# gillesdegottex/percivaltts

Hardware: AMD Instinct MI355X
Metric: acoustic frames/sec per WGAN-GP critic+gen step (higher is better)
Workload: dtype f32

## Files before the change

### include/percival_hip.h

```cpp
#ifndef PERCIVAL_HIP_H
#define PERCIVAL_HIP_H

#include <stddef.h>
#include <stdint.h>

#ifdef __cplusplus
extern "C" {
#endif

#define PTTS_OK            0
#define PTTS_EINVAL       -1
#define PTTS_ELAUNCH      -2
#define PTTS_EWORKSPACE   -3
#define PTTS_EDEVICE      -4

#define PTTS_IN_NONE     0
#define PTTS_IN_LRELU    1
#define PTTS_IN_MASKMUL  2

#define PTTS_PAD_SAME    0
#define PTTS_PAD_CAUSAL  1

#define PTTS_ACT_NONE    0
#define PTTS_ACT_LRELU   1
// ... 126 lines not shown
                                     int Kin, int N, int M, long long lda, long long ldb, int in_mode, float alpha,
                                     void* stream);
int ptts_dense_wgrad_reduce_grouped(const ptts_dense_wgrad_reduce_desc* descs, int n, void* stream);
int ptts_dense_wgrad_bf16x6(const float* A, const float* dY, const float* mask_src, const float* in_scale,
                            const float* in_shift, float* C, float* colsum_b, void* workspace, size_t workspace_bytes,
                            int Kin, int N, int M, long long lda, long long ldb, long long ldc, int in_mode, float alpha,
                            void* stream);
int ptts_dense_bf16x6(const float* A, const void* planes, const float* bias, float* C, int M, int N, int K,
                      long long lda, long long ldc, int in_mode, const float* in_scale, const float* in_shift,
                      const float* mask_src, float alpha, int accumulate, const float* out_mask, void* stream);
int ptts_dense_bf16x6_res(const float* A, const void* planes, const float* bias, float* C, int M, int N, int K,
                          long long lda, long long ldc, int in_mode, const float* in_scale, const float* in_shift,
                          const float* mask_src, float alpha, const float* res, int res_rows, long long ldr,
                          const float* out_mask, void* stream);
int ptts_dense_bf16x6_stats_rows(int M, int N);
int ptts_dense_bf16x6_stats(const float* A, const void* planes, const float* bias, float* C, int M, int N, int K,
                            long long lda, long long ldc, int in_mode, const float* in_scale, const float* in_shift,
                            float alpha, double* stats, int capacity_rows, int* nrows_out, void* stream);
int ptts_dense_bf16x6_bwd_affine(const float* A, const void* planes, float* C, int M, int N, int K, long long lda, long long ldc,
                                 const float* z, const float* scale, const float* shift, float alpha,
                                 double* stats, int capacity_rows, int* nrows_out, void* stream);
int ptts_partial_rows_sum(const double* partials, int nrows, int ncols, double* out, void* stream);
int ptts_dft_mirror(float* Ap, int NB, int B, int Cin, int Kh, void* stream);

int ptts_conv1d_freq_kernel_planes(const float* w, const float* tw, void* planes, int NB, int KW, int Cin, int N, int Kh, void* stream);

int ptts_transpose_batched(const float* src, float* dst, int nb, int rows, int cols, void* stream);
int ptts_conv1d_freq_wgrad_combine(const float* out2, float* dW, int KW, int Cin, int N, int Kh, void* stream);

size_t ptts_conv1d_freq_wgrad_inverse_workspace_bytes(int KW, int Cin, int N);
int ptts_conv1d_freq_wgrad_inverse(const float* Gt, const float* t2, float* dW, void* workspace, size_t workspace_bytes,
                                   int NB, int NBp, int KW, int Cin, int N, int Kh, void* stream);

int ptts_dense_bf16x6_batched(const float* A, long long strideA, const void* planes, long long stride_planes_bytes,
                              const float* bias, float* C, long long strideC, int nbatch, int M, int N, int K,
                              long long lda, long long ldc, int planes_count, void* stream);

int ptts_split3_frames(const float* x, void* p1, void* p2, void* p3, int B, int T, int C, int pad_left, int pad_right,
                       int Cp, void* stream);
int ptts_split3_weight_t(const float* w, void* p1, void* p2, void* p3, int KW, int C, int N, int Cp, void* stream);
int ptts_conv1d_bf16x6(const void* a1, const void* a2, const void* a3, const void* bt1, const void* bt2, const void* bt3,
                       const float* bias, float* y, int B, int T, int KW, int Cp, int N, void* stream);

int ptts_split3_frames_t(const float* x, void* p1, void* p2, void* p3, int B, int T, int C, int pad_left, int Tp, int Crows,
                         long long Pp, void* stream);
int ptts_conv1d_wgrad_bf16x6(const void* xt1, const void* xt2, const void* xt3, const void* yt1, const void* yt2,
                             const void* yt3, float* dw, int B, int T, int KW, int C, int N, int Crows, long long Pp,
                             void* stream);

int ptts_transpose_frames(const float* x, float* out, int B, int T, int C, int pad_left, int Tp, int Crows, long long Pp,
                          void* stream);
int ptts_conv1d_wgrad_t(const float* xt, const float* yt, float* dw, float* db, int B, int T, int KW, int C, int N, int Crows,
                        long long Pp, void* stream);

size_t ptts_colstats_workspace_bytes(long long rows, int C);
int ptts_colstats(const float* x, long long rows, int C,
                  int in_mode, const float* in_scale, const float* in_shift, const float* mask_src, float alpha,
                  double* sums , void* workspace, size_t workspace_bytes, void* stream);

int ptts_bn_finalize(const double* sums, long long count, const float* gamma, const float* beta,
                     float* moving_mean, float* moving_var, float eps, float momentum,
                     int training, int update_moving, int unbiased_moving, int C,
                     float* scale, float* shift, float* mean , float* rstd , void* stream);

int ptts_bn_batch_stats_supported(long long rows, int C);
int ptts_bn_batch_stats(const float* x, long long rows, int C, const float* gamma, const float* beta,
// ... 134 lines not shown
```

### percivaltts_amd/csrc/dense.hip

```cpp
#include "common.h"
#include <cstdlib>

namespace ptts {
namespace dns {

typedef __bf16 bf16x8 __attribute__((ext_vector_type(8)));
typedef __bf16 bf16x4 __attribute__((ext_vector_type(4)));
typedef __bf16 bf16x2 __attribute__((ext_vector_type(2)));
typedef float f32x4 __attribute__((ext_vector_type(4)));
typedef float f32x2 __attribute__((ext_vector_type(2)));
typedef unsigned u32x2 __attribute__((ext_vector_type(2)));
typedef unsigned short u16;

constexpr int THREADS = 512;
constexpr int NBLK = 256;
constexpr int BK = 32;

#define DNS_PRODUCTS(X) X(2, 0) X(1, 1) X(0, 2) X(1, 0) X(0, 1) X(0, 0)
#define DNS_PRODUCTS_NPL(NPL, X) do { if (NPL == 3) { X(2, 0) X(1, 1) X(0, 2) X(1, 0) X(0, 1) } X(0, 0) } while (0)

__device__ __forceinline__ unsigned pk_bf16(float a, float b) {
    return __builtin_bit_cast(unsigned, __builtin_convertvector((f32x2){a, b}, bf16x2));
}
__device__ __forceinline__ void split3_pair(float a, float b, unsigned& p1, unsigned& p2, unsigned& p3) {
    p1 = pk_bf16(a, b);
    const float ra = a - __builtin_bit_cast(float, p1 << 16), rb = b - __builtin_bit_cast(float, p1 & 0xffff0000u);
    p2 = pk_bf16(ra, rb);
    const float sa = ra - __builtin_bit_cast(float, p2 << 16), sb = rb - __builtin_bit_cast(float, p2 & 0xffff0000u);
    p3 = pk_bf16(sa, sb);
}
__device__ __forceinline__ float max_fast(float a, float b) {
    float r;
    asm("v_max_f32 %0, %1, %2" : "=v"(r) : "v"(a), "v"(b));
    return r;
}

__global__ __launch_bounds__(256) void split3_dense_weight_kernel(const float* __restrict__ w, long long ldw, int K, int N,
                                                                  int transposed, u16* __restrict__ planes, int NT, int KS) {
    const long long idx = (long long)blockIdx.x * 256 + threadIdx.x;
    if (idx >= (long long)NT * KS * 64) return;
    const int lane = (int)(idx & 63);
    const long long t = idx >> 6;
    const int ks = (int)(t % KS), nt = (int)(t / KS);
    const int n = nt * 16 + (lane & 15), k0 = ks * 32 + (lane >> 4) * 8;
// ... 151 lines not shown
    const int li = lane & 15, lg = lane >> 4;
#pragma unroll
    for (int j = 0; j < 4; ++j) {
        const int ntl = wave + 4 * j;
        const int nt = cb * 16 + ntl;
        if (nt >= a.NT) continue;
        float v[8];
#pragma unroll
        for (int e = 0; e < 8; ++e) v[e] = tile[(8 * lg + e) * SPL_ROW + 16 * ntl + li];
        unsigned q[3][4];
#pragma unroll
        for (int h = 0; h < 4; ++h) split3_pair(v[2 * h], v[2 * h + 1], q[0][h], q[1][h], q[2][h]);
        const size_t idx = ((size_t)nt * a.KS + ks) * 64 + lane;
#pragma unroll
        for (int p = 0; p < 3; ++p)
            *reinterpret_cast<uint4*>(planes + p * ps + idx * 8) = make_uint4(q[p][0], q[p][1], q[p][2], q[p][3]);
    }
}

#ifndef DNS_DEPTH
#define DNS_DEPTH 2
#endif
struct DenseArgs {
    const float* A; const float* mask_src; const float* in_scale; const float* in_shift;
    const u16* planes; const float* bias; const float* out_mask; float* C;
    int M, N, K, NT, KS;
    long long lda, ldc;
    float alpha, out_alpha;
    int accumulate, has_affine, vec_out;
    const float* res; int res_rows; long long ldr;
    long long bsA, bsP, bsC;
    double* stats;
    const float* om_scale; const float* om_shift;
};

template <int MODE, bool AFFINE, int MT, int NPL>
__global__ __launch_bounds__(THREADS) void dense_bf16x6_kernel(DenseArgs g) {
    if (gridDim.z > 1) {
        g.A += (long long)blockIdx.z * g.bsA;
        g.planes += (long long)blockIdx.z * g.bsP;
        g.C += (long long)blockIdx.z * g.bsC;
    }
    constexpr int TBM = 16 * MT;
    constexpr int NA = (TBM * 8 + THREADS - 1) / THREADS;
    constexpr int ROWS = NA * THREADS / 8;
    constexpr int PL = ROWS * BK;
    constexpr bool MASK = MODE == PTTS_IN_MASKMUL;
    __shared__ __attribute__((aligned(16))) u16 As[2][NPL * PL];
    const int tid = threadIdx.x, lane = tid & 63;
    const int wave = __builtin_amdgcn_readfirstlane(tid >> 6);
    const int li = lane & 15, lg = lane >> 4;
    const int m0 = blockIdx.x * TBM, n0 = blockIdx.y * NBLK;
    const int KS = g.KS;
    const bool wave_live = n0 + 32 * wave < g.N;

    const int kq = tid & 7;
    const float* pa[NA]; const float* pm[NA]; bool oka[NA]; int dst[NA];
#pragma unroll
    for (int j = 0; j < NA; ++j) {
        const int row = (tid + j * THREADS) >> 3;
        oka[j] = row < TBM && m0 + row < g.M;
        const long long base = (long long)(oka[j] ? m0 + row : 0) * g.lda + 4 * kq;
        pa[j] = g.A + base;
        pm[j] = MASK ? g.mask_src + base : nullptr;
        dst[j] = row * BK + ((((kq >> 1) ^ ((row >> 1) & 2))) << 3) + (kq & 1) * 4;
    }
    struct Stage { f32x4 va[NA], vm[MASK ? NA : 1], sc, sh; bool kok; };
    auto load_a = [&](int s, Stage& sg) {
        const int k = s * BK + 4 * kq;
        sg.kok = k < g.K;
        const int ko = sg.kok ? s * BK : -4 * kq;
#pragma unroll
        for (int j = 0; j < NA; ++j) {
            sg.va[j] = *reinterpret_cast<const f32x4*>(pa[j] + ko);
            if (MASK) sg.vm[j] = *reinterpret_cast<const f32x4*>(pm[j] + ko);
        }
        if (AFFINE) {
            sg.sc = *reinterpret_cast<const f32x4*>(g.in_scale + (sg.kok ? k : 0));
            sg.sh = *reinterpret_cast<const f32x4*>(g.in_shift + (sg.kok ? k : 0));
        }
    };
    auto commit = [&](const Stage& sg, u16* as) {
        const f32x4 z4 = {0.f, 0.f, 0.f, 0.f};
#pragma unroll
        for (int j = 0; j < NA; ++j) {
            f32x4 a = sg.va[j];
            if (MODE == PTTS_IN_LRELU) {
                if (AFFINE) a = a * sg.sc + sg.sh;
                if (!(oka[j] && sg.kok)) a = z4;
#pragma unroll
                for (int e = 0; e < 4; ++e) a[e] = max_fast(a[e], g.alpha * a[e]);
            } else if (MASK) {
                if (!(oka[j] && sg.kok)) a = z4;
#pragma unroll
                for (int e = 0; e < 4; ++e) a[e] = a[e] * (sg.vm[j][e] > 0.f ? 1.f : g.alpha);
            } else {
                if (!(oka[j] && sg.kok)) a = z4;
            }
            u16* d = as + dst[j];
            if (NPL == 3) {
                unsigned a1, a2, a3, b1, b2, b3;
                split3_pair(a[0], a[1], a1, a2, a3);
                split3_pair(a[2], a[3], b1, b2, b3);
                *reinterpret_cast<u32x2*>(d) = (u32x2){a1, b1};
                *reinterpret_cast<u32x2*>(d + PL) = (u32x2){a2, b2};
                *reinterpret_cast<u32x2*>(d + 2 * PL) = (u32x2){a3, b3};
            } else {
                *reinterpret_cast<u32x2*>(d) = (u32x2){pk_bf16(a[0], a[1]), pk_bf16(a[2], a[3])};
            }
        }
    };

    const size_t ps = (size_t)g.NT * KS * 512;
    const u16* wp[2];
#pragma unroll
    for (int j = 0; j < 2; ++j) wp[j] = g.planes + (((size_t)((n0 >> 4) + 2 * (wave_live ? wave : 0) + j) * KS) * 64 + lane) * 8;
    auto load_w = [&](int s, bf16x8 (&wf)[2][NPL]) {
#pragma unroll
        for (int j = 0; j < 2; ++j)
#pragma unroll
            for (int p = 0; p < NPL; ++p) wf[j][p] = *reinterpret_cast<const bf16x8*>(wp[j] + p * ps + (size_t)s * 512);
    };

    f32x4 acc[MT][2];
#pragma unroll
    for (int i = 0; i < MT; ++i) { acc[i][0] = f32x4{0.f, 0.f, 0.f, 0.f}; acc[i][1] = f32x4{0.f, 0.f, 0.f, 0.f}; }
    const int boff = li * BK + ((lg ^ ((li >> 1) & 2)) << 3);
    auto mfma_rows = [&](const u16* as, const bf16x8 (&wf)[2][NPL], int i0, int i1) {
#pragma unroll
        for (int i = i0; i < i1; ++i) {
            bf16x8 bf[NPL];
#pragma unroll
            for (int p = 0; p < NPL; ++p) bf[p] = *reinterpret_cast<const bf16x8*>(as + p * PL + boff + i * 16 * BK);
#define DNS_MM(PA, PW)                                                                                    \
            acc[i][0] = __builtin_amdgcn_mfma_f32_16x16x32_bf16(wf[0][PW < NPL ? PW : 0], bf[PA < NPL ? PA : 0], acc[i][0], 0, 0, 0);    \
            acc[i][1] = __builtin_amdgcn_mfma_f32_16x16x32_bf16(wf[1][PW < NPL ? PW : 0], bf[PA < NPL ? PA : 0], acc[i][1], 0, 0, 0);
            DNS_PRODUCTS_NPL(NPL, DNS_MM);
#undef DNS_MM
        }
    };

    constexpr int DEPTH = DNS_DEPTH;
    Stage sg[DEPTH];
    bf16x8 wc[2][NPL], wn[2][NPL];
#pragma unroll
    for (int j = 0; j < DEPTH; ++j) load_a(j, sg[j]);
    load_w(0, wc);
    commit(sg[0], As[0]);
    load_a(DEPTH, sg[0]);
    __syncthreads();
    auto step = [&](int s, int cut, Stage& nx) {
        const u16* as = As[s & 1];
        load_w(s + 1 < KS ? s + 1 : s, wn);
        mfma_rows(as, wc, 0, cut);
        commit(nx, As[(s + 1) & 1]);
        load_a(s + 1 + DEPTH, nx);
        mfma_rows(as, wc, cut, MT);
#pragma unroll
        for (int j = 0; j < 2; ++j)
#pragma unroll
            for (int p = 0; p < NPL; ++p) wc[j][p] = wn[j][p];
        __syncthreads();
    };
    auto run = [&](int cut) {
        int s = 0;
        for (; s + DEPTH <= KS; s += DEPTH) {
#pragma unroll
            for (int j = 0; j < DEPTH; ++j) step(s + j, cut, sg[(j + 1) % DEPTH]);
        }
#pragma unroll
        for (int j = 0; j < DEPTH; ++j)
            if (s + j < KS) step(s + j, cut, sg[(j + 1) % DEPTH]);
    };
    if (wave < 4) run(2); else run(MT - 2);
    if (!wave_live) return;
    const bool interior = m0 + TBM <= g.M;
    if (!g.vec_out) {
#pragma unroll
        for (int j = 0; j < 2; ++j)
#pragma unroll
            for (int i = 0; i < MT; ++i) {
                const int m = m0 + 16 * i + li;
                if (m >= g.M) continue;
#pragma unroll
                for (int e = 0; e < 4; ++e) {
// ... 455 lines not shown
}
extern "C" int ptts_dense_bf16x6_stats_rows(int M, int N) {
    if (M <= 0 || N <= 0) return 0;
    const int mt = pick_mt(M, (N + NBLK - 1) / NBLK);
    return (M + 16 * mt - 1) / (16 * mt);
}

static int dense_launch(const float* A, const void* planes, const float* bias, float* C, int M, int N, int K,
                        long long lda, long long ldc, int in_mode, const float* in_scale, const float* in_shift,
                        const float* mask_src, float alpha, const float* res, int res_rows, long long ldr,
                        const float* out_mask, double* stats, int stats_capacity_rows, int* stats_rows_out, void* stream) {
    const int accumulate = res != nullptr;
    PTTS_REQUIRE(!res || (res_rows > 0 && ldr >= N && M <= 8LL * res_rows), "dense_bf16x6: bad residual (rows %d, ldr %lld)", res_rows, ldr);
    PTTS_REQUIRE(A && planes && C, "dense_bf16x6: null matrix");
    PTTS_REQUIRE(ptts_dense_bf16x6_supported(M, N, K, lda, ldc), "dense_bf16x6: unsupported shape M=%d N=%d K=%d lda=%lld ldc=%lld (K and lda must be multiples of 4)", M, N, K, lda, ldc);
    PTTS_REQUIRE(lda >= K && ldc >= N, "dense_bf16x6: bad leading dims");
    PTTS_REQUIRE(in_mode >= 0 && in_mode <= 2, "dense_bf16x6: bad in_mode %d", in_mode);
    PTTS_REQUIRE((in_scale == nullptr) == (in_shift == nullptr), "dense_bf16x6: scale/shift must come together");
    PTTS_REQUIRE(in_mode != PTTS_IN_MASKMUL || mask_src, "dense_bf16x6: MASKMUL needs mask_src");
    PTTS_REQUIRE(in_mode == PTTS_IN_LRELU || !in_scale, "dense_bf16x6: scale/shift need PTTS_IN_LRELU");
    PTTS_REQUIRE(!(out_mask && bias), "dense_bf16x6: out_mask with bias is not defined");
    PTTS_REQUIRE(alpha >= 0.f && alpha <= 1.f, "dense_bf16x6: LeakyReLU slope %g outside [0, 1]", alpha);
    const bool vec_out = N % 4 == 0 && ldc % 4 == 0 && ((uintptr_t)C & 15) == 0 && (!bias || ((uintptr_t)bias & 15) == 0) &&
                         (!out_mask || ((uintptr_t)out_mask & 15) == 0) && (!res || (((uintptr_t)res & 15) == 0 && ldr % 4 == 0));
    PTTS_REQUIRE(((uintptr_t)A & 15) == 0 && (!mask_src || ((uintptr_t)mask_src & 15) == 0) &&
                 (!in_scale || (((uintptr_t)in_scale | (uintptr_t)in_shift) & 15) == 0), "dense_bf16x6: A, its mask and scale/shift must be 16-byte aligned");
    DenseArgs g;
    g.A = A; g.mask_src = mask_src; g.in_scale = in_scale; g.in_shift = in_shift; g.planes = (const u16*)planes; g.bias = bias;
    g.out_mask = out_mask; g.C = C; g.M = M; g.N = N; g.K = K;
    g.NT = (N + NBLK - 1) / NBLK * (NBLK / 16); g.KS = (K + BK - 1) / BK;
    g.lda = lda; g.ldc = ldc; g.alpha = alpha; g.out_alpha = alpha; g.accumulate = accumulate; g.has_affine = in_scale != nullptr; g.vec_out = vec_out;
    g.res = res; g.res_rows = res ? res_rows : 1; g.ldr = ldr;
    g.bsA = g.bsP = g.bsC = 0;
    const int cb = (N + NBLK - 1) / NBLK;
    const int mt = pick_mt(M, cb);
    const dim3 grid((unsigned)((M + 16 * mt - 1) / (16 * mt)), (unsigned)cb);
    g.stats = stats;
    g.om_scale = g_om_scale; g.om_shift = g_om_shift;
    if (stats) {
        PTTS_REQUIRE(vec_out, "dense_bf16x6_stats: N and ldc must be multiples of 4, C (and bias) 16-byte aligned");
        PTTS_REQUIRE(stats_capacity_rows >= (int)grid.x, "dense_bf16x6_stats: room for %d rows of sums, %d needed", stats_capacity_rows, (int)grid.x);
        *stats_rows_out = (int)grid.x;
    }
    hipStream_t st = (hipStream_t)stream;
    const bool one = ptts::bf16_products();
#define DNS_L(MODE, AFF, MT) do { if (one) hipLaunchKernelGGL((dense_bf16x6_kernel<MODE, AFF, MT, 1>), grid, dim3(THREADS), 0, st, g); \
                                  else hipLaunchKernelGGL((dense_bf16x6_kernel<MODE, AFF, MT, 3>), grid, dim3(THREADS), 0, st, g); } while (0)
#define DNS_M(MT)                                                                \
    do {                                                                         \
        if (in_mode == PTTS_IN_LRELU) { if (in_scale) DNS_L(PTTS_IN_LRELU, true, MT); else DNS_L(PTTS_IN_LRELU, false, MT); } \
        else if (in_mode == PTTS_IN_MASKMUL) DNS_L(PTTS_IN_MASKMUL, false, MT);  \
        else DNS_L(PTTS_IN_NONE, false, MT);                                     \
    } while (0)
    switch (mt) {
        case 4: DNS_M(4); break;
        case 5: DNS_M(5); break;
        case 6: DNS_M(6); break;
        case 7: DNS_M(7); break;
        default: DNS_M(8); break;
    }
#undef DNS_M
#undef DNS_L
    return check_launch("dense_bf16x6");
}

extern "C" int ptts_conv1d_freq_kernel_planes(const float* w, const float* tw, void* planes, int NB, int KW, int Cin, int N, int Kh,
                                              void* stream) {
    PTTS_REQUIRE(w && tw && planes && NB > 0 && Cin > 0 && N > 0, "conv1d_freq_kernel_planes: bad arguments");
    PTTS_REQUIRE(Kh >= Cin && Kh % 8 == 0, "conv1d_freq_kernel_planes: Kh=%d must be a multiple of 8 and >= Cin=%d", Kh, Cin);
    const int NT = (N + NBLK - 1) / NBLK * (NBLK / 16), KS = (2 * Kh + BK - 1) / BK;
    const long long total = (long long)NT * KS * 64;
    const long long fstride = (long long)(ptts_dense_planes_bytes(N, 2 * Kh) / sizeof(u16));
    const dim3 grid((unsigned)((total + 255) / 256), (unsigned)((NB + WDFT_FCH - 1) / WDFT_FCH));
#define WDFT(KWv) hipLaunchKernelGGL(conv1d_wdft_planes_kernel<KWv>, grid, dim3(256), 0, (hipStream_t)stream, w, tw, (u16*)planes, fstride, NB, Cin, N, Kh, NT, KS)
    switch (KW) {
        case 3: WDFT(3); break;
        case 5: WDFT(5); break;
        case 7: WDFT(7); break;
        case 9: WDFT(9); break;
        case 11: WDFT(11); break;
        case 21: WDFT(21); break;
        default: set_error("conv1d_freq_kernel_planes: KW=%d not instantiated (3, 5, 7, 9, 11, 21)", KW); return PTTS_EINVAL;
    }
#undef WDFT
    return check_launch("conv1d_freq_kernel_planes");
}

extern "C" int ptts_dense_bf16x6_batched(const float* A, long long strideA, const void* planes, long long stride_planes_bytes,
                                         const float* bias, float* C, long long strideC, int nbatch, int M, int N, int K,
                                         long long lda, long long ldc, int planes_count, void* stream) {
    PTTS_REQUIRE(A && planes && C && nbatch > 0 && nbatch <= 65535, "dense_bf16x6_batched: bad arguments");
    PTTS_REQUIRE(ptts_dense_bf16x6_supported(M, N, K, lda, ldc), "dense_bf16x6_batched: unsupported shape M=%d N=%d K=%d lda=%lld ldc=%lld", M, N, K, lda, ldc);
    PTTS_REQUIRE(lda >= K && ldc >= N && planes_count >= 1 && planes_count <= 3 && planes_count != 2, "dense_bf16x6_batched: bad leading dims / planes");
    PTTS_REQUIRE(stride_planes_bytes % 16 == 0 && strideA % 4 == 0 && ((uintptr_t)A & 15) == 0, "dense_bf16x6_batched: strides of A / planes must keep 16-byte alignment");
    const bool vec_out = N % 4 == 0 && ldc % 4 == 0 && strideC % 4 == 0 && ((uintptr_t)C & 15) == 0 && (!bias || ((uintptr_t)bias & 15) == 0);
    DenseArgs g;
    g.A = A; g.mask_src = nullptr; g.in_scale = nullptr; g.in_shift = nullptr; g.planes = (const u16*)planes; g.bias = bias;
    g.out_mask = nullptr; g.C = C; g.M = M; g.N = N; g.K = K;
    g.NT = (N + NBLK - 1) / NBLK * (NBLK / 16); g.KS = (K + BK - 1) / BK;
    g.lda = lda; g.ldc = ldc; g.alpha = 0.f; g.out_alpha = 0.f; g.accumulate = 0; g.has_affine = 0; g.vec_out = vec_out;
    g.res = nullptr; g.res_rows = 1; g.ldr = 0;
    g.bsA = strideA; g.bsP = stride_planes_bytes / 2; g.bsC = strideC;
    g.stats = nullptr; g.om_scale = g.om_shift = nullptr;
    const int cb = (N + NBLK - 1) / NBLK;
    int mt = 8; double best_eff = -1.0;
    {
        static int forced = -1;
        if (forced < 0) { const char* e = getenv("PTTS_DENSE_BATCHED_MT"); forced = e ? atoi(e) : 0; }
        for (int m = 8; m >= 4; --m) {
            const int tiles = (M + 16 * m - 1) / (16 * m);
            const double eff = (double)M / (double)(tiles * 16 * m);
            if (eff > best_eff + 1e-9) { best_eff = eff; mt = m; }
        }
        if (forced >= 4 && forced <= 8) mt = forced;
    }
    const dim3 grid((unsigned)((M + 16 * mt - 1) / (16 * mt)), (unsigned)cb, (unsigned)nbatch);
    hipStream_t st = (hipStream_t)stream;
    const bool one = planes_count == 1;
#define DNS_B(MT) do { if (one) hipLaunchKernelGGL((dense_bf16x6_kernel<PTTS_IN_NONE, false, MT, 1>), grid, dim3(THREADS), 0, st, g); \
                       else hipLaunchKernelGGL((dense_bf16x6_kernel<PTTS_IN_NONE, false, MT, 3>), grid, dim3(THREADS), 0, st, g); } while (0)
    switch (mt) {
        case 4: DNS_B(4); break;
        case 5: DNS_B(5); break;
        case 6: DNS_B(6); break;
        case 7: DNS_B(7); break;
        default: DNS_B(8); break;
    }
#undef DNS_B
    return check_launch("dense_bf16x6_batched");
}

extern "C" int ptts_dense_wgrad_bf16x6_supported(int Kin, int N, int M, long long lda, long long ldb) {
    return (Kin > 0 && N > 0 && M > 0 && Kin % 4 == 0 && N % 4 == 0 && lda % 4 == 0 && ldb % 4 == 0 &&
            (long long)((Kin + WT - 1) / WT) * ((N + WT - 1) / WT) <= 65535) ? 1 : 0;
}

namespace {
int wgrad_split(int Kin, int N, int M) {
    const int tiles = ((Kin + WT - 1) / WT) * ((N + WT - 1) / WT), steps = (M + 31) / 32;
    int split = (256 + tiles - 1) / tiles;
    static int env_split = -1;
    if (env_split < 0) { const char* e = getenv("PTTS_DENSE_WGRAD_SPLIT"); env_split = e ? atoi(e) : 0; }
    if (env_split > 0) split = env_split;
    if (split > steps) split = steps;
    return split < 1 ? 1 : split;
}
}

extern "C" size_t ptts_dense_wgrad_workspace_bytes(int Kin, int N, int M) {
    if (Kin <= 0 || N <= 0 || M <= 0) return 0;
    const size_t tiles = (size_t)((Kin + WT - 1) / WT) * ((N + WT - 1) / WT);
    return tiles * wgrad_split(Kin, N, M) * WPART * sizeof(float);
}

extern "C" int ptts_dense_wgrad_bf16x6_partials(const float* A, const float* dY, const float* mask_src, const float* in_scale,
                                                const float* in_shift, void* workspace, size_t workspace_bytes, int* split_out,
                                                int Kin, int N, int M, long long lda, long long ldb, int in_mode, float alpha,
                                                void* stream) {
    PTTS_REQUIRE(A && dY && workspace && split_out, "dense_wgrad_bf16x6: null pointer");
    PTTS_REQUIRE(ptts_dense_wgrad_bf16x6_supported(Kin, N, M, lda, ldb), "dense_wgrad_bf16x6: unsupported shape Kin=%d N=%d M=%d lda=%lld ldb=%lld", Kin, N, M, lda, ldb);
    PTTS_REQUIRE(lda >= Kin && ldb >= N, "dense_wgrad_bf16x6: bad leading dims");
// ... 73 lines not shown
```

### percivaltts_amd/ops.py

```python
import contextlib
import ctypes
import os

import torch

from . import _hip
from ._hip import call, ptr, stream, f32c, _workspace
from .ops_offline import *

IN_NONE, IN_LRELU, IN_MASKMUL = 0, 1, 2
PAD_SAME, PAD_CAUSAL = 0, 1
ACT_NONE, ACT_LRELU, ACT_SIGMOID, ACT_TANH = 0, 1, 2, 3
ACT_CODES = {None: ACT_NONE, 'linear': ACT_NONE, 'lrelu': ACT_LRELU, 'sigmoid': ACT_SIGMOID, 'tanh': ACT_TANH}


class Lazy(object):
    __slots__ = ('z', 'scale', 'shift', 'lrelu', 'alpha')

    def __init__(self, z, scale=None, shift=None, lrelu=False, alpha=0.3):
        self.z, self.scale, self.shift, self.lrelu, self.alpha = z, scale, shift, lrelu, alpha

    @property
    def shape(self):
        return self.z.shape

    def tensor(self):
        if self.scale is None and not self.lrelu:
            return self.z
        return affine_act(self.z, self.scale, self.shift, 'lrelu' if self.lrelu else None, self.alpha)


def as_lazy(v):
    return v if isinstance(v, Lazy) else Lazy(v)


def as_tensor(v):
    return v.tensor() if isinstance(v, Lazy) else v


def _fusable(lz):
    if lz.lrelu:
        return IN_LRELU, lz.scale, lz.shift
    if lz.scale is None:
# ... 1257 lines not shown
        Crows = (C + 63) // 64 * 64
        key = None if src is None else (src._version, tuple(src.shape), KW, _hip.stream_id())
        if src is not None and cls.src is src and cls.key == key:
            return cls.planes
        xt = torch.empty((Crows, Pp), dtype=torch.float32, device=ap.device)
        call('ptts_transpose_frames', ptr(ap), ptr(xt), B, Tp, C, 0, Tp, Crows, Pp, stream(), tag=(B, Tp, C))
        out = (xt, Crows, Pp)
        if src is not None:
            cls.src, cls.key, cls.planes = src, key, out
        return out

    @classmethod
    def clear(cls):
        cls.src = cls.key = cls.planes = None


def clear_caches():
    _C1Split.clear()
    _C1FFT.clear()
    _C1WgradT.clear()
    _C2M.clear()
    _C2C.clear()
    _DenseSplit.clear()
    _C1Cache.key = _C1Cache.ap = _C1Cache.y = None


class _C1FFT(object):
    default = os.environ.get('PTTS_CONV1D_FFT', '1') == '1'
    enabled = default
    KWS = (3, 5, 7, 9, 11, 21)
    wgrad_enabled = os.environ.get('PTTS_CONV1D_FFT_WGRAD', '1') == '1'
    bf16_one_product = os.environ.get('PTTS_CONV1D_FFT_BF16', '1') == '1'
    seg_target = int(os.environ.get('PTTS_CONV1D_FFT_SEG', '100'))
    consts = {}
    x_src = None; x_key = None; x_hat = None
    xw_src = None; xw_key = None; xw_planes = None
    w_hat = {}
    bufs = {}

    @staticmethod
    def eligible(a, w):
        B, T, Cin = a.shape
        KW, _, N = w.shape
        if not (a.is_cuda and B * T >= 4096 and KW >= 3 and KW % 2 == 1 and T % 4 == 0 and N % 4 == 0 and Cin >= 64):
            return False
        return B * (T // _C1FFT.segment(T, KW)) <= 65535

    @classmethod
    def segment(cls, T, KW):
        tgt = cls.seg_target
        if tgt <= 0:
            return T
        best = T
        for S in range(4, T + 1, 4):
            if T % S == 0 and S >= 2 * KW and abs(S - tgt) < abs(best - tgt):
                best = S
        return best

    @classmethod
    def _buf(cls, name, key, nfloats, dev):
        sid = _hip.stream_id()
        k = (name, key, sid)
        t = cls.bufs.get(k)
        if t is None:
            for k2 in [k2 for k2 in cls.bufs if k2[0] == name and k2[2] == sid]:
                del cls.bufs[k2]
            t = cls.bufs[k] = torch.zeros(nfloats, dtype=torch.float32, device=dev)
        return t

    @classmethod
    def _scratch(cls, name, nbytes, dev):
        k = ('scratch', name, _hip.stream_id())
        t = cls.bufs.get(k)
        if t is None or t.numel() < nbytes:
            t = cls.bufs[k] = torch.empty(int(nbytes), dtype=torch.uint8, device=dev)
        return t

    @classmethod
    def const(cls, T, KW, Cin, dev):
# ... 12 lines not shown
        th = 2.0 * math.pi * torch.remainder(f * i, P) / P
        D = torch.stack([torch.cos(th), -torch.sin(th)], dim=1).reshape(2 * NB, P)
        cf = torch.full((NB,), 2.0, dtype=torch.float64); cf[0] = 1.0; cf[P // 2] = 1.0
        R = 2 * NB
        Rp = (R + 3) // 4 * 4
        E = torch.zeros(S, Rp, dtype=torch.float64)
        E[:, 0:R:2] = (torch.cos(th[:, :S]) * cf.view(NB, 1) / P).t()
        E[:, 1:R:2] = (-torch.sin(th[:, :S]) * cf.view(NB, 1) / P).t()
        k = torch.arange(KW, dtype=torch.float64).view(1, KW)
        tk = 2.0 * math.pi * torch.remainder(f * k, P) / P
        Tw = torch.stack([torch.cos(tk), torch.sin(tk)], dim=1).reshape(R, KW)
        NBp = (NB + 3) // 4 * 4
        T2 = torch.zeros(2 * KW, NBp, dtype=torch.float64)
        T2[:KW, :NB] = (torch.cos(tk) * cf.view(NB, 1) / P).t()
        T2[KW:, :NB] = (torch.sin(tk) * cf.view(NB, 1) / P).t()
        TP = (2 * KW + 15) // 16 * 16
        T2f = torch.zeros(NB, TP, dtype=torch.float64)
        T2f[:, :2 * KW] = T2[:, :NB].t()
        to = lambda m: m.to(torch.float32).to(dev).contiguous()
        c = {'S': S, 'NS': NS, 'P': P, 'NB': NB, 'R': R, 'Rp': Rp, 'NBp': NBp, 'TP': TP, 'pl': pl, 'Kh': (Cin + 7) // 8 * 8,
             'D': to(D), 'E': to(E), 'Tw': to(Tw), 'T2': to(T2), 'T2f': to(T2f)}
        cls.consts[key] = c
        return c

    @classmethod
    def x_transform(cls, a, KW):
        B, T, Cin = a.shape
        key = (a._version, tuple(a.shape), KW, _hip.stream_id())
        if cls.x_src is a and cls.x_key == key:
            return cls.x_hat
        c = cls.const(T, KW, Cin, a.device)
        NB, Kh, NS, S, P = c['NB'], c['Kh'], c['NS'], c['S'], c['P']
        Z = B * NS
        Ap = cls._buf('Ap', (B, T, Cin, KW, S), NB * 2 * Z * 2 * Kh, a.device)
        lib = _hip.lib()
        npb = lib.ptts_dense_planes_bytes(Cin, P)
        xpl = cls._scratch('xpl', Z * npb, a.device)
        call('ptts_split3_frame_windows', ptr(a), B, T, Cin, NS, S, -c['pl'], P, P, ptr(xpl), npb, stream(), tag=('x', Z))
        call('ptts_dense_bf16x6_batched', ptr(c['D']), 0, ptr(xpl), npb, None, ptr(Ap), 2 * Kh, Z, c['R'], Cin, P, P, Z * 2 * Kh, 3, stream(),
             tag=('dft', Z, c['R'], Cin, P))
        call('ptts_dft_mirror', ptr(Ap), NB, Z, Cin, Kh, stream())
        cls.x_src, cls.x_key, cls.x_hat = a, key, Ap
        return Ap

    @classmethod
    def kernel(cls, w, T):
        KW, Cin, N = w.shape
        flat = getattr(w, '_ptts_flat', None)
        epoch = None if flat is None else flat.epoch
        sid = _hip.stream_id()
        c = cls.const(T, KW, Cin, w.device)
        NB, Kh = c['NB'], c['Kh']
        geo = (c['S'], NB, Kh)
        ent = cls.w_hat.get((id(w), sid))
        if ent is not None and ent[0] is w and ent[1] == w._version and ent[2] == epoch and flat is not None and ent[5] == geo:
            if cls.frozen_log is not None and id(flat) in cls.frozen:
                cls.frozen_log.append((w, ent[4], T))
            return ent[4]
        lib = _hip.lib()
        npb = lib.ptts_dense_planes_bytes(N, 2 * Kh)
        if ent is not None and ent[0] is w and ent[5] == geo:
            planes = ent[4]
        else:
            planes = torch.empty(NB * npb, dtype=torch.uint8, device=w.device)
        cls._build_kernel_planes(w, c, planes)
        if len(cls.w_hat) >= 8 and (id(w), sid) not in cls.w_hat:
            cls.w_hat = {k: e for k, e in cls.w_hat.items() if id(getattr(e[0], '_ptts_flat', None)) in cls.frozen}
        cls.w_hat[(id(w), sid)] = (w, w._version, epoch, None, planes, geo, T)
        return planes

    @classmethod
    def _build_kernel_planes(cls, w, c, planes):
        KW, Cin, N = w.shape
        NB, Kh = c['NB'], c['Kh']
        if KW in cls.KWS:
            call('ptts_conv1d_freq_kernel_planes', ptr(w), ptr(c['Tw']), ptr(planes), NB, KW, Cin, N, Kh, stream(), tag=(NB, KW, Cin, N))
        else:
            npb = _hip.lib().ptts_dense_planes_bytes(N, 2 * Kh)
            What = torch.zeros(c['R'] * Kh * N, dtype=torch.float32, device=w.device)
            gemm_raw(c['Tw'], w.view(KW, Cin * N), What, c['R'], Cin * N, KW, lda=KW, ldb=Cin * N, ldc=Kh * N)
            call('ptts_split3_dense_weight_strided', ptr(What), 2 * Kh * N, ptr(planes), npb, NB, N, 2 * Kh, N, 0, stream(), tag=('w', NB))

    frozen = set()
    frozen_log = None

    @classmethod
    def refresh_planes(cls, items):
        for w, planes, T in items:
            KW, Cin, N = w.shape
            cls._build_kernel_planes(w, cls.const(T, KW, Cin, w.device), planes)
        return len(items)

    @classmethod
    def forward(cls, a, w, b, y):
        B, T, Cin = a.shape
        KW, _, N = w.shape
        c = cls.const(T, KW, Cin, a.device)
        NB, Kh, NS, S = c['NB'], c['Kh'], c['NS'], c['S']
        Z = B * NS
        lib = _hip.lib()
        Ap = cls.x_transform(a, KW)
        wpl = cls.kernel(w, T)
        npw = lib.ptts_dense_planes_bytes(N, 2 * Kh)
        Yh = cls._scratch('Yh', NB * 2 * Z * N * 4, a.device)
        call('ptts_dense_bf16x6_batched', ptr(Ap), 2 * Z * 2 * Kh, ptr(wpl), npw, None, ptr(Yh), 2 * Z * N, NB, 2 * Z, N, 2 * Kh,
             2 * Kh, N, 1 if _Flags.bf16_products else 3, stream(), tag=('freq', NB, 2 * Z, N, 2 * Kh))
        npy = lib.ptts_dense_planes_bytes(N, c['R'])
        ypl = cls._scratch('ypl', Z * npy, a.device)
        call('ptts_split3_dense_weight_strided', ptr(Yh), N, ptr(ypl), npy, Z, Z * N, c['R'], N, 0, stream(), tag=('y', Z))
        call('ptts_dense_bf16x6_batched', ptr(c['E']), 0, ptr(ypl), npy, ptr(b), ptr(y), S * N, Z, S, N, c['Rp'], c['Rp'], N, 3, stream(),
             tag=('idft', Z, S, N, c['Rp']))

    @classmethod
    def has_x(cls, a, KW):
        return a is not None and cls.x_src is a and cls.x_key == (a._version, tuple(a.shape), KW, _hip.stream_id())

    @classmethod
    def wgrad(cls, a, dy, KW):
        B, T, Cin = a.shape
        N = dy.shape[-1]
        c = cls.const(T, KW, Cin, a.device)
        NB, Kh, NS, S, P = c['NB'], c['Kh'], c['NS'], c['S'], c['P']
        Z = B * NS
        lib = _hip.lib()
        dev = a.device
        Ap = cls.x_hat
        npx = lib.ptts_dense_planes_bytes(2 * Kh, 2 * Z)
        if cls.xw_src is not a or cls.xw_key != cls.x_key or cls.xw_planes is None:
            xw = cls._scratch('xw', NB * npx, dev)
            call('ptts_split3_dense_weight_strided', ptr(Ap), 2 * Z * 2 * Kh, ptr(xw), npx, NB, 2 * Kh, 2 * Z, 2 * Kh, 0, stream(), tag=('xw', NB))
            cls.xw_src, cls.xw_key, cls.xw_planes = a, cls.x_key, xw
        npd = lib.ptts_dense_planes_bytes(N, P)
        dpl = cls._scratch('dpl', Z * npd, dev)
        call('ptts_split3_frame_windows', ptr(dy), B, T, N, NS, S, 0, P, S, ptr(dpl), npd, stream(), tag=('dy', Z))
        DYh = cls._scratch('DYh', NB * 2 * Z * N * 4, dev)
        call('ptts_dense_bf16x6_batched', ptr(c['D']), 0, ptr(dpl), npd, None, ptr(DYh), N, Z, c['R'], N, P, P, Z * N, 3, stream(),
             tag=('dft_dy', Z, c['R'], N, P))
        DYt = cls._scratch('DYt', NB * N * 2 * Z * 4, dev)
        call('ptts_transpose_batched', ptr(DYh), ptr(DYt), NB, 2 * Z, N, stream())
        Gt = cls._scratch('Gt', NB * N * 2 * Kh * 4, dev)
        call('ptts_dense_bf16x6_batched', ptr(DYt), N * 2 * Z, ptr(cls.xw_planes), npx, None, ptr(Gt), N * 2 * Kh, NB, N, 2 * Kh, 2 * Z,
             2 * Z, 2 * Kh, 1 if _Flags.bf16_products else 3, stream(), tag=('corr', NB, N, 2 * Kh, 2 * Z))
        dw = torch.empty((KW, Cin, N), dtype=torch.float32, device=dev)
        if KW in cls.KWS:
            ws = _workspace(lib.ptts_conv1d_freq_wgrad_inverse_workspace_bytes(KW, Cin, N), dev)
            call('ptts_conv1d_freq_wgrad_inverse', ptr(Gt), ptr(c['T2f']), ptr(dw), ptr(ws), ws.numel(), NB, c['TP'], KW, Cin, N, Kh, stream(),
                 tag=(NB, KW, Cin, N))
        else:
            out2 = torch.empty(2 * KW * N * 2 * Kh, dtype=torch.float32, device=dev)
            gemm_raw(c['T2'], Gt[:NB * N * 2 * Kh * 4].view(torch.float32), out2, 2 * KW, N * 2 * Kh, NB, lda=c['NBp'], ldb=N * 2 * Kh, ldc=N * 2 * Kh)
            call('ptts_conv1d_freq_wgrad_combine', ptr(out2), ptr(dw), KW, Cin, N, Kh, stream())
        return dw

    @classmethod
    def clear(cls):
        cls.x_src = cls.x_key = cls.x_hat = None
        cls.xw_src = cls.xw_key = cls.xw_planes = None
        cls.w_hat = {k: (e if id(getattr(e[0], '_ptts_flat', None)) in cls.frozen else (e[0], None, None, e[3], e[4], e[5]) + tuple(e[6:]))
                     for k, e in cls.w_hat.items()}


def conv1d_fft(on):
    _C1FFT.enabled = _C1FFT.default if on is None else bool(on)
    _C1FFT.clear()


def conv1d_split(on):
    _C1Split.enabled = _C1Split.default if on is None else bool(on)
    _C1Split.clear()


class Conv1dFn(torch.autograd.Function):
    @staticmethod
    def forward(ctx, a, w, b, pre=None):
        f32c(a, 'conv1d.a'); f32c(w, 'conv1d.w')
        B, T, Cin = a.shape
        KW, Ci2, N = w.shape
        assert Ci2 == Cin
        pl = (KW - 1) // 2
        if pre is not None:
            saved, padded, y = pre
        else:
            y = torch.empty((B, T, N), dtype=torch.float32, device=a.device)
            if _C1FFT.enabled and _C1Split.enabled and (not _Flags.bf16_products or _C1FFT.bf16_one_product) and _C1FFT.eligible(a, w):
                _C1FFT.forward(a, w, b, y)
                saved, padded = a, False
            elif _C1Split.enabled and not _Flags.deterministic and _C1Split.eligible(a, w):
                xp, Cp = _C1Split.frames(a, pl, KW - 1 - pl)
                wp = _C1Split.kernel(w)
# ... 683 lines not shown
```

Before: 4.563 million.

## Store DFT spectra compactly and synthesize mirrored half inside dense GEMM loads

Adds left- and right-mirrored operand forms to the batched bf16x6 dense kernel. The kernel reconstructs the sign-flipped mirrored half of the frequency-domain input on the fly, either while loading A or by offsetting and flipping the weight planes. The FFT conv1d path then stores only half the spectrum when the batch-segment count is a multiple of 32, which skips the dft_mirror pass and halves the Ap buffer and xw plane split. In exchange it adds per-load branching, sign XORs and extra template instantiations in the hot GEMM loops.

After: 4.138 million. -9.3%, worse.

```diff
diff --git a/include/percival_hip.h b/include/percival_hip.h
--- a/include/percival_hip.h
+++ b/include/percival_hip.h
@@ -182,6 +182,8 @@
 int ptts_conv1d_freq_wgrad_inverse(const float* Gt, const float* t2, float* dW, void* workspace, size_t workspace_bytes,
                                    int NB, int NBp, int KW, int Cin, int N, int Kh, void* stream);
 
+#define PTTS_DENSE_LEFT_MIRRORED  0x100
+#define PTTS_DENSE_RIGHT_MIRRORED 0x200
 int ptts_dense_bf16x6_batched(const float* A, long long strideA, const void* planes, long long stride_planes_bytes,
                               const float* bias, float* C, long long strideC, int nbatch, int M, int N, int K,
                               long long lda, long long ldc, int planes_count, void* stream);
diff --git a/percivaltts_amd/csrc/dense.hip b/percivaltts_amd/csrc/dense.hip
--- a/percivaltts_amd/csrc/dense.hip
+++ b/percivaltts_amd/csrc/dense.hip
@@ -10,6 +10,7 @@
 typedef float f32x4 __attribute__((ext_vector_type(4)));
 typedef float f32x2 __attribute__((ext_vector_type(2)));
 typedef unsigned u32x2 __attribute__((ext_vector_type(2)));
+typedef unsigned u32x4 __attribute__((ext_vector_type(4)));
 typedef unsigned short u16;
 
 constexpr int THREADS = 512;
@@ -227,9 +228,10 @@
     long long bsA, bsP, bsC;
     double* stats;
     const float* om_scale; const float* om_shift;
+    int mirZ, mirKh;
 };
 
-template <int MODE, bool AFFINE, int MT, int NPL>
+template <int MODE, bool AFFINE, int MT, int NPL, int FORM = 0>
 __global__ __launch_bounds__(THREADS) void dense_bf16x6_kernel(DenseArgs g) {
     if (gridDim.z > 1) {
         g.A += (long long)blockIdx.z * g.bsA;
@@ -241,6 +243,8 @@
     constexpr int ROWS = NA * THREADS / 8;
     constexpr int PL = ROWS * BK;
     constexpr bool MASK = MODE == PTTS_IN_MASKMUL;
+    constexpr bool LMIR = FORM == 1 || FORM == 2;
+    static_assert(FORM == 0 || (MODE == PTTS_IN_NONE && !AFFINE), "the mirrored forms take no input transform");
     __shared__ __attribute__((aligned(16))) u16 As[2][NPL * PL];
     const int tid = threadIdx.x, lane = tid & 63;
     const int wave = __builtin_amdgcn_readfirstlane(tid >> 6);
@@ -251,6 +255,8 @@
 
     const int kq = tid & 7;
     const float* pa[NA]; const float* pm[NA]; bool oka[NA]; int dst[NA];
+    const float* pa1[LMIR ? NA : 1];
+    unsigned rsgn[LMIR ? NA : 1];
 #pragma unroll
     for (int j = 0; j < NA; ++j) {
         const int row = (tid + j * THREADS) >> 3;
@@ -259,15 +265,23 @@
         pa[j] = g.A + base;
         pm[j] = MASK ? g.mask_src + base : nullptr;
         dst[j] = row * BK + ((((kq >> 1) ^ ((row >> 1) & 2))) << 3) + (kq & 1) * 4;
-    }
-    struct Stage { f32x4 va[NA], vm[MASK ? NA : 1], sc, sh; bool kok; };
+        if (LMIR) {
+            const int m = oka[j] ? m0 + row : 0, p = m >= g.mirZ ? 1 : 0;
+            pa1[j] = pa[j] + (long long)(1 - 2 * p) * g.mirZ * g.lda - g.mirKh;
+            rsgn[j] = p ? 0u : 0x80000000u;
+        }
+    }
+    struct Stage { f32x4 va[NA], vm[MASK ? NA : 1], sc, sh; bool kok, h; };
     auto load_a = [&](int s, Stage& sg) {
         const int k = s * BK + 4 * kq;
         sg.kok = k < g.K;
-        const int ko = sg.kok ? s * BK : -4 * kq;
+        if (FORM == 1) sg.h = s * BK >= g.mirKh;
+        if (FORM == 2) sg.h = sg.kok && k >= g.mirKh;
+        const int ko = sg.kok ? s * BK : (FORM == 1 && sg.h ? g.mirKh : 0) - 4 * kq;
 #pragma unroll
         for (int j = 0; j < NA; ++j) {
-            sg.va[j] = *reinterpret_cast<const f32x4*>(pa[j] + ko);
+            if (LMIR) sg.va[j] = *reinterpret_cast<const f32x4*>((sg.h ? pa1[j] : pa[j]) + ko);
+            else sg.va[j] = *reinterpret_cast<const f32x4*>(pa[j] + ko);
             if (MASK) sg.vm[j] = *reinterpret_cast<const f32x4*>(pm[j] + ko);
         }
         if (AFFINE) {
@@ -291,6 +305,7 @@
                 for (int e = 0; e < 4; ++e) a[e] = a[e] * (sg.vm[j][e] > 0.f ? 1.f : g.alpha);
             } else {
                 if (!(oka[j] && sg.kok)) a = z4;
+                if (LMIR) a = __builtin_bit_cast(f32x4, __builtin_bit_cast(u32x4, a) ^ (sg.h ? rsgn[j] : 0u));
             }
             u16* d = as + dst[j];
             if (NPL == 3) {
@@ -308,13 +323,44 @@
 
     const size_t ps = (size_t)g.NT * KS * 512;
     const u16* wp[2];
-#pragma unroll
-    for (int j = 0; j < 2; ++j) wp[j] = g.planes + (((size_t)((n0 >> 4) + 2 * (wave_live ? wave : 0) + j) * KS) * 64 + lane) * 8;
+    unsigned wo[2] = {0u, 0u};
+    unsigned wfl[2] = {0u, 0u};
+    const int Zs = FORM == 3 ? g.mirZ / BK : 0;
+#pragma unroll
+    for (int j = 0; j < 2; ++j) {
+        const int nt = (n0 >> 4) + 2 * (wave_live ? wave : 0) + j;
+        if (FORM == 3) {
+            const int n = nt * 16 + li;
+            const bool live = n < g.N, h = live && n >= g.mirKh;
+            const int c = live ? n - (h ? g.mirKh : 0) : 0;
+            wo[j] = (unsigned)((((c >> 4) * KS + (h ? Zs : 0)) * 64 + lg * 16 + (c & 15)) * 16);
+            wp[j] = g.planes;
+            wfl[j] = h ? 0x80008000u : 0u;
+        } else {
+            wp[j] = g.planes + (((size_t)nt * KS) * 64 + lane) * 8;
+        }
+    }
+    const bool anyflip = FORM == 3 && __builtin_amdgcn_readfirstlane((int)(__ballot(wfl[0] | wfl[1]) != 0ull)) != 0;
+    auto w_advance = [&](int s) {
+        const unsigned fwd = s + 1 < KS ? 1024u : 0u;
+        const unsigned back = s + 1 == Zs ? (unsigned)(2 * Zs) * 1024u : 0u;
+#pragma unroll
+        for (int j = 0; j < 2; ++j) wo[j] += fwd - (wfl[j] ? back : 0u);
+    };
+    auto flip_w = [&](bf16x8 (&wf)[2][NPL]) {
+#pragma unroll
+        for (int j = 0; j < 2; ++j)
+#pragma unroll
+            for (int p = 0; p < NPL; ++p) wf[j][p] = __builtin_bit_cast(bf16x8, __builtin_bit_cast(u32x4, wf[j][p]) ^ wfl[j]);
+    };
     auto load_w = [&](int s, bf16x8 (&wf)[2][NPL]) {
 #pragma unroll
         for (int j = 0; j < 2; ++j)
 #pragma unroll
-            for (int p = 0; p < NPL; ++p) wf[j][p] = *reinterpret_cast<const bf16x8*>(wp[j] + p * ps + (size_t)s * 512);
+            for (int p = 0; p < NPL; ++p) {
+                if (FORM == 3) wf[j][p] = *reinterpret_cast<const bf16x8*>(reinterpret_cast<const char*>(g.planes + p * ps) + wo[j]);
+                else wf[j][p] = *reinterpret_cast<const bf16x8*>(wp[j] + p * ps + (size_t)s * 512);
+            }
     };
 
     f32x4 acc[MT][2];
@@ -344,8 +390,10 @@
     commit(sg[0], As[0]);
     load_a(DEPTH, sg[0]);
     __syncthreads();
-    auto step = [&](int s, int cut, Stage& nx) {
+    auto step = [&](int s, int cut, Stage& nx) __attribute__((always_inline)) {
         const u16* as = As[s & 1];
+        if (FORM == 3) w_advance(s);
+        if (anyflip && s < Zs) flip_w(wc);
         load_w(s + 1 < KS ? s + 1 : s, wn);
         mfma_rows(as, wc, 0, cut);
         commit(nx, As[(s + 1) & 1]);
@@ -867,6 +915,7 @@
     g.lda = lda; g.ldc = ldc; g.alpha = alpha; g.out_alpha = alpha; g.accumulate = accumulate; g.has_affine = in_scale != nullptr; g.vec_out = vec_out;
     g.res = res; g.res_rows = res ? res_rows : 1; g.ldr = ldr;
     g.bsA = g.bsP = g.bsC = 0;
+    g.mirZ = g.mirKh = 0;
     const int cb = (N + NBLK - 1) / NBLK;
     const int mt = pick_mt(M, cb);
     const dim3 grid((unsigned)((M + 16 * mt - 1) / (16 * mt)), (unsigned)cb);
@@ -924,17 +973,26 @@
 extern "C" int ptts_dense_bf16x6_batched(const float* A, long long strideA, const void* planes, long long stride_planes_bytes,
                                          const float* bias, float* C, long long strideC, int nbatch, int M, int N, int K,
                                          long long lda, long long ldc, int planes_count, void* stream) {
+    const int flags = planes_count & ~0xff;
+    planes_count &= 0xff;
+    const bool left = flags == PTTS_DENSE_LEFT_MIRRORED, right = flags == PTTS_DENSE_RIGHT_MIRRORED;
+    PTTS_REQUIRE(flags == 0 || left || right, "dense_bf16x6_batched: unknown or combined operand flags 0x%x", flags);
     PTTS_REQUIRE(A && planes && C && nbatch > 0 && nbatch <= 65535, "dense_bf16x6_batched: bad arguments");
     PTTS_REQUIRE(ptts_dense_bf16x6_supported(M, N, K, lda, ldc), "dense_bf16x6_batched: unsupported shape M=%d N=%d K=%d lda=%lld ldc=%lld", M, N, K, lda, ldc);
-    PTTS_REQUIRE(lda >= K && ldc >= N && planes_count >= 1 && planes_count <= 3 && planes_count != 2, "dense_bf16x6_batched: bad leading dims / planes");
+    PTTS_REQUIRE(lda >= (left ? K / 2 : K) && ldc >= N && planes_count >= 1 && planes_count <= 3 && planes_count != 2, "dense_bf16x6_batched: bad leading dims / planes");
+    PTTS_REQUIRE(!left || (M % 2 == 0 && K % 8 == 0), "dense_bf16x6_batched: PTTS_DENSE_LEFT_MIRRORED needs an even M and K %% 8 == 0 (M=%d K=%d)", M, K);
+    PTTS_REQUIRE(!right || (N % 2 == 0 && K % (2 * BK) == 0), "dense_bf16x6_batched: PTTS_DENSE_RIGHT_MIRRORED needs an even N and K %% 64 == 0 (N=%d K=%d)", N, K);
     PTTS_REQUIRE(stride_planes_bytes % 16 == 0 && strideA % 4 == 0 && ((uintptr_t)A & 15) == 0, "dense_bf16x6_batched: strides of A / planes must keep 16-byte alignment");
     const bool vec_out = N % 4 == 0 && ldc % 4 == 0 && strideC % 4 == 0 && ((uintptr_t)C & 15) == 0 && (!bias || ((uintptr_t)bias & 15) == 0);
     DenseArgs g;
     g.A = A; g.mask_src = nullptr; g.in_scale = nullptr; g.in_shift = nullptr; g.planes = (const u16*)planes; g.bias = bias;
     g.out_mask = nullptr; g.C = C; g.M = M; g.N = N; g.K = K;
-    g.NT = (N + NBLK - 1) / NBLK * (NBLK / 16); g.KS = (K + BK - 1) / BK;
+    g.NT = ((right ? N / 2 : N) + NBLK - 1) / NBLK * (NBLK / 16); g.KS = (K + BK - 1) / BK;
     g.lda = lda; g.ldc = ldc; g.alpha = 0.f; g.out_alpha = 0.f; g.accumulate = 0; g.has_affine = 0; g.vec_out = vec_out;
     g.res = nullptr; g.res_rows = 1; g.ldr = 0;
+    g.mirZ = left ? M / 2 : right ? K / 2 : 0; g.mirKh = left ? K / 2 : right ? N / 2 : 0;
+    PTTS_REQUIRE(!right || (long long)g.NT * g.KS * 1024 < (1LL << 32), "dense_bf16x6_batched: PTTS_DENSE_RIGHT_MIRRORED addresses a plane by 32-bit offsets (N=%d K=%d)", N, K);
+    const int form = left ? ((K / 2) % BK == 0 ? 1 : 2) : right ? 3 : 0;
     g.bsA = strideA; g.bsP = stride_planes_bytes / 2; g.bsC = strideC;
     g.stats = nullptr; g.om_scale = g.om_shift = nullptr;
     const int cb = (N + NBLK - 1) / NBLK;
@@ -952,8 +1010,9 @@
     const dim3 grid((unsigned)((M + 16 * mt - 1) / (16 * mt)), (unsigned)cb, (unsigned)nbatch);
     hipStream_t st = (hipStream_t)stream;
     const bool one = planes_count == 1;
-#define DNS_B(MT) do { if (one) hipLaunchKernelGGL((dense_bf16x6_kernel<PTTS_IN_NONE, false, MT, 1>), grid, dim3(THREADS), 0, st, g); \
-                       else hipLaunchKernelGGL((dense_bf16x6_kernel<PTTS_IN_NONE, false, MT, 3>), grid, dim3(THREADS), 0, st, g); } while (0)
+#define DNS_F(MT, FORM) do { if (one) hipLaunchKernelGGL((dense_bf16x6_kernel<PTTS_IN_NONE, false, MT, 1, FORM>), grid, dim3(THREADS), 0, st, g); \
+                             else hipLaunchKernelGGL((dense_bf16x6_kernel<PTTS_IN_NONE, false, MT, 3, FORM>), grid, dim3(THREADS), 0, st, g); } while (0)
+#define DNS_B(MT) do { if (form == 1) DNS_F(MT, 1); else if (form == 2) DNS_F(MT, 2); else if (form == 3) DNS_F(MT, 3); else DNS_F(MT, 0); } while (0)
     switch (mt) {
         case 4: DNS_B(4); break;
         case 5: DNS_B(5); break;
@@ -962,6 +1021,7 @@
         default: DNS_B(8); break;
     }
 #undef DNS_B
+#undef DNS_F
     return check_launch("dense_bf16x6_batched");
 }
 
diff --git a/percivaltts_amd/ops.py b/percivaltts_amd/ops.py
--- a/percivaltts_amd/ops.py
+++ b/percivaltts_amd/ops.py
@@ -9,6 +9,7 @@
 from .ops_offline import *
 
 IN_NONE, IN_LRELU, IN_MASKMUL = 0, 1, 2
+DENSE_LEFT_MIRRORED, DENSE_RIGHT_MIRRORED = 0x100, 0x200
 PAD_SAME, PAD_CAUSAL = 0, 1
 ACT_NONE, ACT_LRELU, ACT_SIGMOID, ACT_TANH = 0, 1, 2, 3
 ACT_CODES = {None: ACT_NONE, 'linear': ACT_NONE, 'lrelu': ACT_LRELU, 'sigmoid': ACT_SIGMOID, 'tanh': ACT_TANH}
@@ -1332,8 +1333,9 @@
     wgrad_enabled = os.environ.get('PTTS_CONV1D_FFT_WGRAD', '1') == '1'
     bf16_one_product = os.environ.get('PTTS_CONV1D_FFT_BF16', '1') == '1'
     seg_target = int(os.environ.get('PTTS_CONV1D_FFT_SEG', '100'))
+    min_frames = 4096
     consts = {}
-    x_src = None; x_key = None; x_hat = None
+    x_src = None; x_key = None; x_hat = None; x_compact = False
     xw_src = None; xw_key = None; xw_planes = None
     w_hat = {}
     bufs = {}
@@ -1342,9 +1344,13 @@
     def eligible(a, w):
         B, T, Cin = a.shape
         KW, _, N = w.shape
-        if not (a.is_cuda and B * T >= 4096 and KW >= 3 and KW % 2 == 1 and T % 4 == 0 and N % 4 == 0 and Cin >= 64):
+        if not (a.is_cuda and B * T >= _C1FFT.min_frames and KW >= 3 and KW % 2 == 1 and T % 4 == 0 and N % 4 == 0 and Cin >= 64):
             return False
         return B * (T // _C1FFT.segment(T, KW)) <= 65535
+
+    @classmethod
+    def compact(cls, B, T, KW):
+        return (B * (T // cls.segment(T, KW))) % 32 == 0
 
     @classmethod
     def segment(cls, T, KW):
@@ -1423,15 +1429,18 @@
         c = cls.const(T, KW, Cin, a.device)
         NB, Kh, NS, S, P = c['NB'], c['Kh'], c['NS'], c['S'], c['P']
         Z = B * NS
-        Ap = cls._buf('Ap', (B, T, Cin, KW, S), NB * 2 * Z * 2 * Kh, a.device)
+        compact = cls.compact(B, T, KW)
+        ld = Kh if compact else 2 * Kh
+        Ap = cls._buf('Ap', (B, T, Cin, KW, S, compact), NB * 2 * Z * ld, a.device)
         lib = _hip.lib()
         npb = lib.ptts_dense_planes_bytes(Cin, P)
         xpl = cls._scratch('xpl', Z * npb, a.device)
         call('ptts_split3_frame_windows', ptr(a), B, T, Cin, NS, S, -c['pl'], P, P, ptr(xpl), npb, stream(), tag=('x', Z))
-        call('ptts_dense_bf16x6_batched', ptr(c['D']), 0, ptr(xpl), npb, None, ptr(Ap), 2 * Kh, Z, c['R'], Cin, P, P, Z * 2 * Kh, 3, stream(),
+        call('ptts_dense_bf16x6_batched', ptr(c['D']), 0, ptr(xpl), npb, None, ptr(Ap), ld, Z, c['R'], Cin, P, P, Z * ld, 3, stream(),
              tag=('dft', Z, c['R'], Cin, P))
-        call('ptts_dft_mirror', ptr(Ap), NB, Z, Cin, Kh, stream())
-        cls.x_src, cls.x_key, cls.x_hat = a, key, Ap
+        if not compact:
+            call('ptts_dft_mirror', ptr(Ap), NB, Z, Cin, Kh, stream())
+        cls.x_src, cls.x_key, cls.x_hat, cls.x_compact = a, key, Ap, compact
         return Ap
 
     @classmethod
@@ -1494,8 +1503,9 @@
         wpl = cls.kernel(w, T)
         npw = lib.ptts_dense_planes_bytes(N, 2 * Kh)
         Yh = cls._scratch('Yh', NB * 2 * Z * N * 4, a.device)
-        call('ptts_dense_bf16x6_batched', ptr(Ap), 2 * Z * 2 * Kh, ptr(wpl), npw, None, ptr(Yh), 2 * Z * N, NB, 2 * Z, N, 2 * Kh,
-             2 * Kh, N, 1 if _Flags.bf16_products else 3, stream(), tag=('freq', NB, 2 * Z, N, 2 * Kh))
+        ld, form = (Kh, DENSE_LEFT_MIRRORED) if cls.x_compact else (2 * Kh, 0)
+        call('ptts_dense_bf16x6_batched', ptr(Ap), 2 * Z * ld, ptr(wpl), npw, None, ptr(Yh), 2 * Z * N, NB, 2 * Z, N, 2 * Kh,
+             ld, N, (1 if _Flags.bf16_products else 3) | form, stream(), tag=('freq', NB, 2 * Z, N, 2 * Kh))
         npy = lib.ptts_dense_planes_bytes(N, c['R'])
         ypl = cls._scratch('ypl', Z * npy, a.device)
         call('ptts_split3_dense_weight_strided', ptr(Yh), N, ptr(ypl), npy, Z, Z * N, c['R'], N, 0, stream(), tag=('y', Z))
@@ -1516,10 +1526,11 @@
         lib = _hip.lib()
         dev = a.device
         Ap = cls.x_hat
-        npx = lib.ptts_dense_planes_bytes(2 * Kh, 2 * Z)
+        ld, form = (Kh, DENSE_RIGHT_MIRRORED) if cls.x_compact else (2 * Kh, 0)
+        npx = lib.ptts_dense_planes_bytes(ld, 2 * Z)
         if cls.xw_src is not a or cls.xw_key != cls.x_key or cls.xw_planes is None:
             xw = cls._scratch('xw', NB * npx, dev)
-            call('ptts_split3_dense_weight_strided', ptr(Ap), 2 * Z * 2 * Kh, ptr(xw), npx, NB, 2 * Kh, 2 * Z, 2 * Kh, 0, stream(), tag=('xw', NB))
+            call('ptts_split3_dense_weight_strided', ptr(Ap), 2 * Z * ld, ptr(xw), npx, NB, ld, 2 * Z, ld, 0, stream(), tag=('xw', NB))
             cls.xw_src, cls.xw_key, cls.xw_planes = a, cls.x_key, xw
         npd = lib.ptts_dense_planes_bytes(N, P)
         dpl = cls._scratch('dpl', Z * npd, dev)
@@ -1531,7 +1542,7 @@
         call('ptts_transpose_batched', ptr(DYh), ptr(DYt), NB, 2 * Z, N, stream())
         Gt = cls._scratch('Gt', NB * N * 2 * Kh * 4, dev)
         call('ptts_dense_bf16x6_batched', ptr(DYt), N * 2 * Z, ptr(cls.xw_planes), npx, None, ptr(Gt), N * 2 * Kh, NB, N, 2 * Kh, 2 * Z,
-             2 * Z, 2 * Kh, 1 if _Flags.bf16_products else 3, stream(), tag=('corr', NB, N, 2 * Kh, 2 * Z))
+             2 * Z, 2 * Kh, (1 if _Flags.bf16_products else 3) | form, stream(), tag=('corr', NB, N, 2 * Kh, 2 * Z))
         dw = torch.empty((KW, Cin, N), dtype=torch.float32, device=dev)
         if KW in cls.KWS:
             ws = _workspace(lib.ptts_conv1d_freq_wgrad_inverse_workspace_bytes(KW, Cin, N), dev)
@@ -1546,6 +1557,7 @@
     @classmethod
     def clear(cls):
         cls.x_src = cls.x_key = cls.x_hat = None
+        cls.x_compact = False
         cls.xw_src = cls.xw_key = cls.xw_planes = None
         cls.w_hat = {k: (e if id(getattr(e[0], '_ptts_flat', None)) in cls.frozen else (e[0], None, None, e[3], e[4], e[5]) + tuple(e[6:]))
                      for k, e in cls.w_hat.items()}
```
